# SensorsINI/v2e

Measured on NVIDIA H100. Metric: Mevents/s, higher is better.
Workload: dtype fp16 tensor-core convs (fp32 accumulate) + f64 pixel state

## Files before the change

### include/v2e_b200.h

```cpp
#ifndef V2E_B200_H
#define V2E_B200_H

#include <stdint.h>

#ifdef __cplusplus
extern "C" {
#endif

typedef enum V2eStatus {
    V2E_OK = 0,
    V2E_E_INVALID = -1,
    V2E_E_CUDA = -2,
    V2E_E_CAPACITY = -3,
    V2E_E_ITER_CAP = -4,
    V2E_E_STATE = -5,
    V2E_E_UNSUPPORTED = -6,
    V2E_E_FALLBACK = -7
} V2eStatus;

typedef enum V2eFrameDtype { V2E_U8 = 0, V2E_F32 = 1, V2E_F64 = 2 } V2eFrameDtype;

const char *v2e_last_error(void);
int v2e_version(void);
int v2e_abi_info(int *version, int *emu_cfg_size, int *frame_info_size, int *unet_weights_size);
// ... 131 lines not shown

int v2e_emu_state_is_f64(V2eEmu *h);
void *v2e_emu_state_ptr(V2eEmu *h, int which);

int v2e_emu_draw_noise(V2eEmu *h, uint32_t frame_index, float *leak_randn, float *shot_u01, float *pr_randn,
                       void *stream);


int v2e_conv2d_lrelu_sm100(const void *x1_dev, int C1, const void *x2_dev, int C2,
                           const void *wgt_dev, const float *bias_dev, int Cout_pad, int KH, int KW,
                           int N, int H, int W, void *out_dev, int out_cstride, int out_mode,
                           int co_real, float slope, void *stream);

enum {
    V2E_CONV_TILE_AUTO = -1,
    V2E_CONV_TILE_LEGACY = 0,
    V2E_CONV_TILE_256x128 = 1,
    V2E_CONV_TILE_128x256 = 2
};
int v2e_conv2d_lrelu_sm100_tile(const void *x1_dev, int C1, const void *x2_dev, int C2,
                                const void *wgt_dev, const float *bias_dev, int Cout_pad, int KH, int KW,
                                int N, int H, int W, void *out_dev, int out_cstride, int out_mode,
                                int co_real, float slope, int tile, void *stream);
int v2e_conv_pick_tile(int C1, int C2, int Cout_pad, int KH, int KW, int N, int H, int W, int n_sms);

int v2e_conv2d_lrelu_sm100_strip(const void *x1_dev, int C1, const void *x2_dev, int C2,
                                 const void *wgt_row_dev, const float *bias_dev, int Cout_pad, int KH,
                                 int KW, int N, int H, int W, void *out_dev, int out_cstride,
                                 int out_mode, int co_real, float slope, void *stream);
int v2e_conv_strip_pick_kc(int C1, int C2, int Cout_pad, int KH, int KW, int W);

enum {
    V2E_STRIP_CHAIN_AUTO = -1,
    V2E_STRIP_CHAIN_PAIRED = 0,
    V2E_STRIP_CHAIN_STACKED = 1
};
int v2e_conv2d_lrelu_sm100_strip_chain(const void *x1_dev, int C1, const void *x2_dev, int C2,
                                       const void *wgt_row_dev, const float *bias_dev, int Cout_pad, int KH,
                                       int KW, int N, int H, int W, void *out_dev, int out_cstride,
                                       int out_mode, int co_real, float slope, int chain, void *stream);
int v2e_conv_strip_pick_chain(int C1, int C2, int Cout_pad, int KH, int KW, int W);

int v2e_conv2d_up2_lrelu_sm100(const void *x_low_dev, int C, const void *wgt_fold_dev, const void *wgt_plain_dev,
                               const float *bias_dev, int Cout_pad, int N, int H_out, int W_out, void *out_dev,
                               int out_cstride, float slope, void *stream);
int v2e_conv_up2_fold_weights(const float *w_host, int cout, int cin, int Cout_pad, int C_pad, void *out_host);
// ... 89 lines not shown
```

### v2e_b200/_lib.py

```python
import ctypes
import os

from . import build as _build

_LIB = None


class V2eEmuCfg(ctypes.Structure):
    _fields_ = [
        ("width", ctypes.c_int32), ("height", ctypes.c_int32),
        ("per_pixel_thres", ctypes.c_int32), ("hdr", ctypes.c_int32),
        ("pos_thres_nominal", ctypes.c_double), ("neg_thres_nominal", ctypes.c_double),
        ("cutoff_hz", ctypes.c_double), ("leak_rate_hz", ctypes.c_double),
        ("leak_jitter_fraction", ctypes.c_double), ("refractory_period_s", ctypes.c_double),
        ("shot_noise_rate_hz", ctypes.c_double), ("shot_inten_factor", ctypes.c_double),
        ("rng_mode", ctypes.c_int32), ("iter_cap", ctypes.c_int32),
        ("seed", ctypes.c_uint64),
        ("csdvs", ctypes.c_int32), ("max_frames_per_step", ctypes.c_int32),
        ("cs_tau_p_s", ctypes.c_double), ("cs_tau_h_s", ctypes.c_double),
        ("scidvs", ctypes.c_int32), ("photoreceptor_noise", ctypes.c_int32),
        ("rng_pixel_offset", ctypes.c_uint32), ("full_frame_px", ctypes.c_uint32),
        ("own_row0", ctypes.c_int32), ("own_rows", ctypes.c_int32),
        ("cs_halo_rows", ctypes.c_int32), ("reserved1", ctypes.c_int32),
    ]
# ... 53 lines not shown
    "v2e_emu_first_frame": (_i, [_vp, _vp, _i, _d, _d, _vp]),
    "v2e_emu_step": (_i, [_vp, _vp, _i, _i, _vp, _d, _vp, _vp, _vp, _u64, _u64, _i, _i, _vp]),
    "v2e_emu_collect": (_i, [_vp, ctypes.POINTER(V2eFrameInfo), _i, ctypes.POINTER(_i),
                             ctypes.POINTER(_u64), _vp]),
    "v2e_emu_phase_count": (_i, [_vp, _vp, _i, _d, _d, _vp, _vp, _i, _u64, _u64, _vp]),
    "v2e_emu_phase_update": (_i, [_vp, _vp, _i, _d, _d, _vp, _vp, _u64, _u64, _vp]),
    "v2e_emu_max_n_dev": (_vp, [_vp]),
    "v2e_emu_cs_begin": (_i, [_vp, _vp, _i, _d, _d, _u64, _u64, ctypes.POINTER(_i), _vp]),
    "v2e_emu_cs_pack": (_i, [_vp, _vp]),
    "v2e_emu_cs_unpack_from": (_i, [_vp, _vp, _vp, _vp]),
    "v2e_emu_cs_send_dev": (_vp, [_vp]),
    "v2e_emu_cs_chunk": (_i, [_vp, _i, _i, _vp]),
    "v2e_emu_cs_max_dev": (_vp, [_vp]),
    "v2e_emu_cs_advance": (_i, [_vp, _i, _i, _vp]),
    "v2e_emu_cs_update": (_i, [_vp, _vp, _i, _vp, _vp, _vp]),
    "v2e_emu_phase_filter": (_i, [_vp, _d, _d, _u64, _i, _vp]),
    "v2e_emu_read_counts": (_i, [_vp, ctypes.POINTER(ctypes.c_int32), _vp, _i, _vp]),
    "v2e_emu_phase_shot": (_i, [_vp, _vp, _i, _d, _d, _vp, _u64, _vp]),
    "v2e_emu_phase_emit": (_i, [_vp, _d, _d, _vp, _u64, _vp]),
    "v2e_conv2d_lrelu_sm100": (_i, [_vp, _i, _vp, _i, _vp, _vp, _i, _i, _i, _i, _i, _i, _vp, _i, _i, _i,
                                    ctypes.c_float, _vp]),
    "v2e_conv2d_lrelu_sm100_tile": (_i, [_vp, _i, _vp, _i, _vp, _vp, _i, _i, _i, _i, _i, _i, _vp, _i, _i, _i,
                                         ctypes.c_float, _i, _vp]),
    "v2e_conv_pick_tile": (_i, [_i, _i, _i, _i, _i, _i, _i, _i, _i]),
    "v2e_conv2d_lrelu_sm100_strip": (_i, [_vp, _i, _vp, _i, _vp, _vp, _i, _i, _i, _i, _i, _i, _vp, _i, _i, _i,
                                          ctypes.c_float, _vp]),
    "v2e_conv_strip_pick_kc": (_i, [_i, _i, _i, _i, _i, _i]),
    "v2e_conv2d_lrelu_sm100_strip_chain": (_i, [_vp, _i, _vp, _i, _vp, _vp, _i, _i, _i, _i, _i, _i, _vp, _i, _i, _i,
                                                ctypes.c_float, _i, _vp]),
    "v2e_conv_strip_pick_chain": (_i, [_i, _i, _i, _i, _i, _i]),
    "v2e_conv2d_up2_lrelu_sm100": (_i, [_vp, _i, _vp, _vp, _vp, _i, _i, _i, _i, _vp, _i, ctypes.c_float, _vp]),
    "v2e_conv_up2_fold_weights": (_i, [_vp, _i, _i, _i, _i, _vp]),
    "v2e_conv_up2_supported_c": (_i, [_i, _i, _i]),
    "v2e_slomo_create": (_i, [_i, _i, _i, _vp, _vp, ctypes.POINTER(_vp)]),
    "v2e_slomo_destroy": (_i, [_vp]),
    "v2e_slomo_set_pairs": (_i, [_vp, _vp, _i, _vp]),
    "v2e_slomo_max_flow": (_i, [_vp, ctypes.POINTER(ctypes.c_float), _vp]),
    "v2e_slomo_interp": (_i, [_vp, _d, _vp, _vp, _vp]),
    "v2e_slomo_set_option": (_i, [_vp, _i, _i]),
    "v2e_slomo_check_finite": (_i, [_vp, ctypes.POINTER(_i), _vp]),
    "v2e_slomo_profile": (_i, [_vp, _i]),
    "v2e_slomo_profile_read": (_i, [_vp, ctypes.POINTER(ctypes.c_float), ctypes.POINTER(_i),
                                    ctypes.POINTER(ctypes.c_double), _vp]),
    "v2e_slomo_profile_read_layers": (_i, [_vp, ctypes.POINTER(ctypes.c_float), ctypes.POINTER(_i),
                                           ctypes.POINTER(ctypes.c_double), ctypes.POINTER(ctypes.c_float),
                                           ctypes.POINTER(_i), ctypes.POINTER(ctypes.c_double), _vp]),
# ... 98 lines not shown
```

### v2e_b200/csrc/conv_tc.cu

```cuda
#include <cuda.h>
#include <cuda_fp16.h>
#include <cuda_runtime.h>
#include <math.h>
#include <stdint.h>
#include <stdio.h>
#include <string.h>
#include <vector>

#include "../../include/v2e_b200.h"
#include "common.cuh"
#include "tc_common.cuh"

namespace {

constexpr int kTileH = 8, kTileW = 16, kBM = kTileH * kTileW;
constexpr int kStages = 4;
constexpr int kConvThreads = 288;
constexpr int kProducerWarp = 8;
constexpr int kConsumerWarps = 8;

struct ConvParams {
    int N, H, W;
    int C1, C2;
    int KH, KW;
    int KC;
    int BN;
    int stages;
    int co_fast;
    int tiles_x, tiles_y;
    int n_tiles;
    int out_cstride;
    int out_mode;
    int co_real;
    float slope;
    const float *bias;
    void *out;
};

__device__ __forceinline__ uint8_t *align1024(uint8_t *p) { return (uint8_t *)(((uintptr_t)p + 1023) & ~(uintptr_t)1023); }

__device__ __forceinline__ float lrelu(float x, float slope) { return x > 0.f ? x : x * slope; }

template <int BN>
__device__ __forceinline__ void epilogue_row(const float (&d)[BN / 2], int i, bool inb, size_t pix, int lane,
                                             const float *bias, float slope, int out_mode, void *out, int cstride,
                                             int co0, __half2 (&h)[BN / 8]) {
#pragma unroll
    for (int j = 0; j < BN / 8; j++) {
        const int c = 8 * j + 2 * (lane & 3);
        const float x0 = lrelu(d[4 * j + 2 * i] + __ldg(bias + c), slope);
        const float x1 = lrelu(d[4 * j + 2 * i + 1] + __ldg(bias + c + 1), slope);
        h[j] = __floats2half2_rn(x0, x1);
        if (inb) {
            if (out_mode == 0) *(__half2 *)((__half *)out + pix * cstride + co0 + c) = h[j];
            else if (j == 0) *(float2 *)((float *)out + pix * 8 + c) = make_float2(x0, x1);
        }
    }
}

template <int BN>
__global__ void __launch_bounds__(kConvThreads, 1)
conv_tc_kernel(const __grid_constant__ CUtensorMap tmA, const __grid_constant__ CUtensorMap tmA2,
               const __grid_constant__ CUtensorMap tmB, const ConvParams p) {
    extern __shared__ __align__(1024) uint8_t smem_raw[];
    uint8_t *smem = align1024(smem_raw);
    const uint32_t a_bytes = kBM * p.KC * 2;
    const uint32_t b_bytes_raw = BN * p.KC * 2;
    const uint32_t b_bytes = (b_bytes_raw + 1023) & ~1023u;
    const uint32_t stage_bytes = a_bytes + b_bytes;
    __shared__ __align__(8) uint64_t full_bar[kStages], empty_bar[kStages];

    const int warp = threadIdx.x >> 5, lane = threadIdx.x & 31;
    const int tile = p.co_fast ? blockIdx.y : blockIdx.x;
    const int tx = tile % p.tiles_x, ty = (tile / p.tiles_x) % p.tiles_y, n = tile / (p.tiles_x * p.tiles_y);
    const int x0 = tx * kTileW, y0 = ty * kTileH;
    const int n0 = (p.co_fast ? blockIdx.x : blockIdx.y) * BN;
    const int Ctot = p.C1 + p.C2;
    const int slabs = Ctot / p.KC;
    const int k_iters = p.KH * p.KW * slabs;

    if (threadIdx.x == 0) {
        for (int s = 0; s < kStages; s++) { mbar_init(&full_bar[s], 1); mbar_init(&empty_bar[s], kConsumerWarps); }
        fence_barrier_init();
    }
    if (warp == kProducerWarp && lane == 0) {
        prefetch_tmap(&tmA);
        if (p.C2) prefetch_tmap(&tmA2);
        prefetch_tmap(&tmB);
    }
    __syncthreads();

    if (warp == kProducerWarp) {
        if (lane == 0) {
            int stage = 0;
            uint32_t phase = 0;
            const int ph = p.KH / 2, pw = p.KW / 2;
            for (int tap = 0; tap < p.KH * p.KW; tap++) {
                const int r = tap / p.KW, s = tap % p.KW;
                for (int sl = 0; sl < slabs; sl++) {
                    mbar_wait(&empty_bar[stage], phase ^ 1);
                    uint8_t *sa = smem + stage * stage_bytes, *sb = sa + a_bytes;
                    mbar_expect_tx(&full_bar[stage], a_bytes + b_bytes_raw);
                    const int c = sl * p.KC;
                    if (c < p.C1) tma_load_4d(sa, &tmA, &full_bar[stage], c, x0 + s - pw, y0 + r - ph, n);
                    else tma_load_4d(sa, &tmA2, &full_bar[stage], c - p.C1, x0 + s - pw, y0 + r - ph, n);
                    tma_load_2d(sb, &tmB, &full_bar[stage], tap * Ctot + c, n0);
                    if (++stage == p.stages) { stage = 0; phase ^= 1; }
                }
            }
        }
    } else {
        const int g = warp >> 2;
        const uint64_t d0 = make_smem_desc(smem_u32(smem), swizzle_layout(p.KC), 8u * p.KC * 2u);
        const uint32_t stage16 = stage_bytes >> 4, a16 = a_bytes >> 4, half16 = (64u * p.KC * 2u) >> 4;
        const int ksteps = p.KC / 16;
        float acc[BN / 2];
#pragma unroll
        for (int i = 0; i < BN / 2; i++) acc[i] = 0.f;
        int stage = 0, prev = -1;
        uint32_t phase = 0;
        for (int it = 0; it < k_iters; it++) {
            mbar_wait(&full_bar[stage], phase);
            const uint32_t base = (uint32_t)stage * stage16;
            wgmma_fence();
            for (int j = 0; j < ksteps; j++)
                wgmma_f16<BN>(acc, desc_add(d0, base + (uint32_t)g * half16 + 2u * j), desc_add(d0, base + a16 + 2u * j),
                              (uint32_t)((it | j) != 0));
            wgmma_commit();
            wgmma_wait<1>();
            if (prev >= 0) { __syncwarp(); if (lane == 0) mbar_arrive(&empty_bar[prev]); }
            prev = stage;
            if (++stage == p.stages) { stage = 0; phase ^= 1; }
        }
        wgmma_wait<0>();
        wgmma_fence_regs(acc);
        __half2 hv[BN / 8];
#pragma unroll
        for (int i = 0; i < 2; i++) {
            const int m = 64 * g + 16 * (warp & 3) + (lane >> 2) + 8 * i;
            const int py = y0 + m / kTileW, px = x0 + m % kTileW;
            const bool inb = py < p.H && px < p.W;
            const size_t pix = ((size_t)n * p.H + py) * p.W + px;
            epilogue_row<BN>(acc, i, inb, pix, lane, p.bias + n0, p.slope, p.out_mode, p.out, p.out_cstride, n0, hv);
        }
    }
}

template <int MH, int BN>
__global__ void __launch_bounds__(kConvThreads, 1)
conv_wide_kernel(const __grid_constant__ CUtensorMap tmA, const __grid_constant__ CUtensorMap tmA2,
                 const __grid_constant__ CUtensorMap tmB, const ConvParams p) {
    constexpr int TH = kTileH * MH, BM = kBM * MH;
    extern __shared__ __align__(1024) uint8_t smem_raw[];
    uint8_t *smem = align1024(smem_raw);
    const uint32_t a_bytes = BM * p.KC * 2;
    const uint32_t b_bytes = BN * p.KC * 2;
    const uint32_t stage_bytes = a_bytes + b_bytes;
    __shared__ __align__(8) uint64_t full_bar[kStages], empty_bar[kStages];

    const int warp = threadIdx.x >> 5, lane = threadIdx.x & 31;
    const int tile = p.co_fast ? blockIdx.y : blockIdx.x;
    const int tx = tile % p.tiles_x, ty = (tile / p.tiles_x) % p.tiles_y, n = tile / (p.tiles_x * p.tiles_y);
    const int x0 = tx * kTileW, y0 = ty * TH;
    const int n0 = (p.co_fast ? blockIdx.x : blockIdx.y) * BN;
    const int Ctot = p.C1 + p.C2;
    const int slabs = Ctot / p.KC;
    const int k_iters = p.KH * p.KW * slabs;

    if (threadIdx.x == 0) {
        for (int s = 0; s < kStages; s++) { mbar_init(&full_bar[s], 1); mbar_init(&empty_bar[s], kConsumerWarps); }
        fence_barrier_init();
    }
    if (warp == kProducerWarp && lane == 0) {
        prefetch_tmap(&tmA);
        if (p.C2) prefetch_tmap(&tmA2);
        prefetch_tmap(&tmB);
    }
    __syncthreads();

    if (warp == kProducerWarp) {
        if (lane == 0) {
            int stage = 0;
            uint32_t phase = 0;
            const int ph = p.KH / 2, pw = p.KW / 2;
            for (int tap = 0; tap < p.KH * p.KW; tap++) {
                const int r = tap / p.KW, s = tap % p.KW;
                for (int sl = 0; sl < slabs; sl++) {
                    mbar_wait(&empty_bar[stage], phase ^ 1);
                    uint8_t *sa = smem + stage * stage_bytes, *sb = sa + a_bytes;
                    mbar_expect_tx(&full_bar[stage], a_bytes + b_bytes);
                    const int c = sl * p.KC;
                    if (c < p.C1) tma_load_4d(sa, &tmA, &full_bar[stage], c, x0 + s - pw, y0 + r - ph, n);
                    else tma_load_4d(sa, &tmA2, &full_bar[stage], c - p.C1, x0 + s - pw, y0 + r - ph, n);
                    tma_load_2d(sb, &tmB, &full_bar[stage], tap * Ctot + c, n0);
                    if (++stage == p.stages) { stage = 0; phase ^= 1; }
                }
            }
        }
    } else {
        const int g = __shfl_sync(0xffffffffu, warp >> 2, 0);
        const uint64_t d0 = make_smem_desc(smem_u32(smem), swizzle_layout(p.KC), 8u * p.KC * 2u);
        const uint32_t stage16 = stage_bytes >> 4, a16 = a_bytes >> 4, q16 = (64u * p.KC * 2u) >> 4;
        const int ksteps = p.KC / 16;
        float acc[MH][BN / 2];
#pragma unroll
        for (int h = 0; h < MH; h++) {
#pragma unroll
            for (int i = 0; i < BN / 2; i++) acc[h][i] = 0.f;
            wgmma_fence_regs(acc[h]);
        }
        int stage = 0, prev = -1;
        uint32_t phase = 0;
        for (int it = 0; it < k_iters; it++) {
            mbar_wait(&full_bar[stage], phase);
            const uint32_t base = (uint32_t)stage * stage16;
            wgmma_fence();
            for (int j = 0; j < ksteps; j++) {
#pragma unroll
                for (int h = 0; h < MH; h++)
                    wgmma_f16<BN>(acc[h], desc_add(d0, base + (uint32_t)(g * MH + h) * q16 + 2u * j),
                                  desc_add(d0, base + a16 + 2u * j), (uint32_t)((it | j) != 0));
            }
            wgmma_commit();
            wgmma_wait<1>();
            if (prev >= 0) { __syncwarp(); if (lane == 0) mbar_arrive(&empty_bar[prev]); }
            prev = stage;
            if (++stage == p.stages) { stage = 0; phase ^= 1; }
        }
        wgmma_wait<0>();
#pragma unroll
        for (int h = 0; h < MH; h++) wgmma_fence_regs(acc[h]);
        const float *bias = p.bias + n0;
        __half *out = (__half *)p.out + n0;
#pragma unroll
        for (int h = 0; h < MH; h++) {
            size_t pix[2];
            bool inb[2];
#pragma unroll
            for (int i = 0; i < 2; i++) {
                const int m = 64 * (g * MH + h) + 16 * (warp & 3) + (lane >> 2) + 8 * i;
                const int py = y0 + m / kTileW, px = x0 + m % kTileW;
                inb[i] = py < p.H && px < p.W;
                pix[i] = (((size_t)n * p.H + py) * p.W + px) * p.out_cstride;
            }
#pragma unroll
            for (int j = 0; j < BN / 8; j++) {
                const int c = 8 * j + 2 * (lane & 3);
                const float2 b = __ldg((const float2 *)(bias + c));
#pragma unroll
                for (int i = 0; i < 2; i++)
                    if (inb[i])
                        *(__half2 *)(out + pix[i] + c) = __floats2half2_rn(lrelu(acc[h][4 * j + 2 * i] + b.x, p.slope),
                                                                           lrelu(acc[h][4 * j + 2 * i + 1] + b.y, p.slope));
            }
        }
    }
}


constexpr int kRowTile = 128;

struct StripParams {
    int N, H, W;
    int C1, C2;
    int KH, KW;
    int KC, BN;
    int tiles_x, seg_h, n_seg, n_items;
    int nslot;
    void *pool_out;
    int pool_cstride;
    int n_split, cout_pad;
    int slab_bytes;
    int w_bytes;
    int out_cstride, out_mode, co_real;
    float slope;
    const float *bias;
    void *out;
};
constexpr int kMaxSlot = 12;
constexpr int kStripThreads = 288;

// ... 507 lines not shown
    const int kc = v2e_conv_pick_kc(C1, C2);
    if (n_sms < 1) n_sms = 1;
    int best = V2E_CONV_TILE_LEGACY;
    double best_cost = 0.0;
    for (int tile = V2E_CONV_TILE_LEGACY; tile <= V2E_CONV_TILE_128x256; tile++) {
        int mh, bn;
        tile_shape(tile, Cout_pad, &mh, &bn);
        const bool wide = tile != V2E_CONV_TILE_LEGACY;
        if (wide && (kc != 64 || Cout_pad % bn || (tile == V2E_CONV_TILE_256x128) != (Cout_pad == 128))) continue;
        long tiles = (long)((W + kTileW - 1) / kTileW) * ((H + kTileH * mh - 1) / (kTileH * mh)) * N;
        const long ctas = tiles * (Cout_pad / bn);
        const long waves = (ctas + n_sms - 1) / n_sms;
        const double a_bytes = (double)kBM * mh * kc * 2, b_bytes = (double)bn * kc * 2;
        const double flops = 2.0 * kBM * mh * bn * kc;
        const double per_stage = fmax((a_bytes + b_bytes) / 24.0, flops / 4096.0);
        const double cost = (double)waves * per_stage;
        if (tile == V2E_CONV_TILE_LEGACY || cost < best_cost) { best = tile; best_cost = cost; }
    }
    return best;
}

struct V2eConvLaunch {
    CUtensorMap tmA, tmA2, tmB;
    ConvParams p;
    dim3 grid;
    int mh;
    size_t smem;
};

int v2e_conv_prepare(V2eConvLaunch *L, const void *x1, int C1, const void *x2, int C2, const void *wgt,
                     const float *bias, int Cout_pad, int KH, int KW, int N, int H, int W, void *out,
                     int out_cstride, int out_mode, int co_real, float slope, int tile, int n_sms) {
    if (C1 % 16 || C2 % 16 || !(Cout_pad == 16 || Cout_pad == 32 || Cout_pad == 64 || (Cout_pad > 0 && Cout_pad % 128 == 0)))
        return v2e_set_error(V2E_E_INVALID, "conv: channel counts must be padded to 16 (Cout to 16/32/64/128k)%s", "");
    if (tile == V2E_CONV_TILE_AUTO) tile = v2e_conv_pick_tile(C1, C2, Cout_pad, KH, KW, N, H, W, n_sms);
    if (tile < V2E_CONV_TILE_LEGACY || tile > V2E_CONV_TILE_128x256)
        return v2e_set_error(V2E_E_INVALID, "conv: unknown tile%s", "");
    memset(L, 0, sizeof(*L));
    ConvParams &p = L->p;
    int mh, bn;
    tile_shape(tile, Cout_pad, &mh, &bn);
    const bool wide = tile != V2E_CONV_TILE_LEGACY;
    p.N = N; p.H = H; p.W = W; p.C1 = C1; p.C2 = C2; p.KH = KH; p.KW = KW;
    p.KC = v2e_conv_pick_kc(C1, C2);
    p.BN = bn;
    if (wide && (Cout_pad % bn || out_mode != 0))
        return v2e_set_error(V2E_E_INVALID, "conv: the wide tiles need fp16 output and Cout_pad a multiple of their width%s", "");
    p.stages = kStages;
    p.tiles_x = (W + kTileW - 1) / kTileW;
    p.tiles_y = (H + kTileH * mh - 1) / (kTileH * mh);
    p.n_tiles = p.tiles_x * p.tiles_y * N;
    p.out_cstride = out_cstride; p.out_mode = out_mode; p.co_real = co_real; p.slope = slope;
    p.bias = bias; p.out = out;
    L->mh = mh;
    int rc;
    if ((rc = make_act_tmap_h(&L->tmA, x1, N, H, W, C1, p.KC, kTileH * mh))) return rc;
    if (C2) { if ((rc = make_act_tmap_h(&L->tmA2, x2, N, H, W, C2, p.KC, kTileH * mh))) return rc; }
    else L->tmA2 = L->tmA;
    if ((rc = v2e_make_wgt_tmap(&L->tmB, wgt, Cout_pad, KH * KW * (C1 + C2), p.KC, bn))) return rc;
    const unsigned tiles = (unsigned)p.n_tiles, cob = (unsigned)(Cout_pad / p.BN);
    p.co_fast = (cob > 1 && tiles <= 65535u) ? 1 : 0;
    L->grid = p.co_fast ? dim3(cob, tiles, 1) : dim3(tiles, cob, 1);
    size_t stage = (size_t)kBM * mh * p.KC * 2 + (((size_t)p.BN * p.KC * 2 + 1023) & ~(size_t)1023);
    L->smem = stage * p.stages + 1024;
    return V2E_OK;
}

template <int BN>
static cudaError_t conv_launch_bn(const V2eConvLaunch *L, cudaStream_t st) {
    static PerDeviceOnce attr_once;
    if (attr_once.first()) cudaFuncSetAttribute(conv_tc_kernel<BN>, cudaFuncAttributeMaxDynamicSharedMemorySize, 200 * 1024);
    conv_tc_kernel<BN><<<L->grid, kConvThreads, L->smem, st>>>(L->tmA, L->tmA2, L->tmB, L->p);
    return cudaGetLastError();
}

template <int MH, int BN>
static cudaError_t conv_launch_wide(const V2eConvLaunch *L, cudaStream_t st) {
    static PerDeviceOnce attr_once;
    if (attr_once.first())
        cudaFuncSetAttribute(conv_wide_kernel<MH, BN>, cudaFuncAttributeMaxDynamicSharedMemorySize, 226 * 1024);
    conv_wide_kernel<MH, BN><<<L->grid, kConvThreads, L->smem, st>>>(L->tmA, L->tmA2, L->tmB, L->p);
    return cudaGetLastError();
}

int v2e_conv_launch(const V2eConvLaunch *L, cudaStream_t st) {
    cudaError_t e;
    if (L->mh == 2 && L->p.BN == 128) e = conv_launch_wide<2, 128>(L, st);
    else if (L->mh == 1 && L->p.BN == 256) e = conv_launch_wide<1, 256>(L, st);
    else switch (L->p.BN) {
        case 16: e = conv_launch_bn<16>(L, st); break;
        case 32: e = conv_launch_bn<32>(L, st); break;
        case 64: e = conv_launch_bn<64>(L, st); break;
        case 128: e = conv_launch_bn<128>(L, st); break;
        default: return v2e_set_error(V2E_E_UNSUPPORTED, "conv_tc_kernel: unsupported tile width%s", "");
    }
    if (e != cudaSuccess) return v2e_set_error(V2E_E_CUDA, "conv_tc_kernel launch: %s", cudaGetErrorString(e));
    return V2E_OK;
}

size_t v2e_conv_launch_size(void) { return sizeof(V2eConvLaunch); }

static int device_sms() {
    int dev = 0, sms = 132;
    cudaGetDevice(&dev);
    cudaDeviceGetAttribute(&sms, cudaDevAttrMultiProcessorCount, dev);
    return sms;
}

extern "C" int v2e_conv2d_lrelu_sm100_tile(const void *x1_dev, int C1, const void *x2_dev, int C2,
                                           const void *wgt_dev, const float *bias_dev, int Cout_pad, int KH, int KW,
                                           int N, int H, int W, void *out_dev, int out_cstride, int out_mode,
                                           int co_real, float slope, int tile, void *stream) {
    V2eConvLaunch L;
    int rc = v2e_conv_prepare(&L, x1_dev, C1, x2_dev, C2, wgt_dev, bias_dev, Cout_pad, KH, KW, N, H, W, out_dev,
                              out_cstride, out_mode, co_real, slope, tile, device_sms());
    if (rc) return rc;
    return v2e_conv_launch(&L, (cudaStream_t)stream);
}

extern "C" int v2e_conv2d_lrelu_sm100(const void *x1_dev, int C1, const void *x2_dev, int C2,
                                      const void *wgt_dev, const float *bias_dev, int Cout_pad, int KH, int KW,
                                      int N, int H, int W, void *out_dev, int out_cstride, int out_mode,
                                      int co_real, float slope, void *stream) {
    return v2e_conv2d_lrelu_sm100_tile(x1_dev, C1, x2_dev, C2, wgt_dev, bias_dev, Cout_pad, KH, KW, N, H, W, out_dev,
                                       out_cstride, out_mode, co_real, slope, V2E_CONV_TILE_AUTO, stream);
}

struct V2eStripLaunch {
    CUtensorMap tmA, tmA2, tmB;
    StripParams p;
    int stacked;
    int grid;
    size_t smem;
};

static int make_rowseg_tmap(CUtensorMap *tm, const void *ptr, int N, int H, int W, int C, int KC, int KW) {
    EncodeTiledFn fn = encode_fn();
    if (!fn) return v2e_set_error(V2E_E_CUDA, "cuTensorMapEncodeTiled unavailable%s", "");
    cuuint64_t dims[4] = {(cuuint64_t)C, (cuuint64_t)W, (cuuint64_t)H, (cuuint64_t)N};
    cuuint64_t strides[3] = {(cuuint64_t)C * 2, (cuuint64_t)W * C * 2, (cuuint64_t)H * W * C * 2};
// ... 336 lines not shown
```

### v2e_b200/csrc/tc_common.cuh

```cuda
#pragma once
#include <cuda.h>
#include <cuda_runtime.h>
#include <stdint.h>

__device__ __forceinline__ uint32_t smem_u32(const void *p) { return (uint32_t)__cvta_generic_to_shared(p); }

__device__ __forceinline__ void mbar_init(uint64_t *bar, uint32_t count) {
    asm volatile("mbarrier.init.shared::cta.b64 [%0], %1;" ::"r"(smem_u32(bar)), "r"(count) : "memory");
}
__device__ __forceinline__ void fence_barrier_init() { asm volatile("fence.mbarrier_init.release.cluster;" ::: "memory"); }
__device__ __forceinline__ void fence_proxy_async() { asm volatile("fence.proxy.async.shared::cta;" ::: "memory"); }
__device__ __forceinline__ void mbar_expect_tx(uint64_t *bar, uint32_t bytes) {
    asm volatile("mbarrier.arrive.expect_tx.shared::cta.b64 _, [%0], %1;" ::"r"(smem_u32(bar)), "r"(bytes) : "memory");
}
__device__ __forceinline__ void mbar_arrive(uint64_t *bar) {
    asm volatile("mbarrier.arrive.shared::cta.b64 _, [%0];" ::"r"(smem_u32(bar)) : "memory");
}
__device__ __forceinline__ void mbar_wait(uint64_t *bar, uint32_t parity) {
    const uint32_t addr = smem_u32(bar);
    uint32_t done;
    do {
        asm volatile(
            "{\n\t.reg .pred p;\n\t"
            "mbarrier.try_wait.parity.shared::cta.b64 p, [%1], %2;\n\t"
            "selp.u32 %0, 1, 0, p;\n\t}"
            : "=r"(done) : "r"(addr), "r"(parity) : "memory");
    } while (!done);
}

__device__ __forceinline__ void prefetch_tmap(const CUtensorMap *tm) {
    asm volatile("prefetch.tensormap [%0];" ::"l"((uint64_t)tm) : "memory");
}
__device__ __forceinline__ void tma_load_4d(void *dst, const CUtensorMap *tm, uint64_t *bar, int c0, int c1, int c2, int c3) {
    asm volatile(
        "cp.async.bulk.tensor.4d.shared::cluster.global.tile.mbarrier::complete_tx::bytes [%0], [%1, {%3, %4, %5, %6}], [%2];"
        ::"r"(smem_u32(dst)), "l"((uint64_t)tm), "r"(smem_u32(bar)), "r"(c0), "r"(c1), "r"(c2), "r"(c3) : "memory");
}
__device__ __forceinline__ void tma_load_2d(void *dst, const CUtensorMap *tm, uint64_t *bar, int c0, int c1) {
    asm volatile(
        "cp.async.bulk.tensor.2d.shared::cluster.global.tile.mbarrier::complete_tx::bytes [%0], [%1, {%3, %4}], [%2];"
        ::"r"(smem_u32(dst)), "l"((uint64_t)tm), "r"(smem_u32(bar)), "r"(c0), "r"(c1) : "memory");
}

__device__ __forceinline__ uint32_t elect_one() {
    uint32_t pred;
    asm volatile("{\n\t.reg .pred p;\n\telect.sync _|p, 0xffffffff;\n\tselp.u32 %0, 1, 0, p;\n\t}" : "=r"(pred));
    return pred;
}

__device__ __forceinline__ void wgmma_fence() { asm volatile("wgmma.fence.sync.aligned;" ::: "memory"); }
__device__ __forceinline__ void wgmma_commit() { asm volatile("wgmma.commit_group.sync.aligned;" ::: "memory"); }
template <int N>
__device__ __forceinline__ void wgmma_wait() { asm volatile("wgmma.wait_group.sync.aligned %0;" ::"n"(N) : "memory"); }
template <int R>
__device__ __forceinline__ void wgmma_fence_regs(float (&d)[R]) {
#pragma unroll
    for (int i = 0; i < R; i++) asm volatile("" : "+f"(d[i])::"memory");
}

__device__ __forceinline__ void wgmma_m64n16k16(float (&d)[8], uint64_t adesc, uint64_t bdesc, uint32_t scale_d) {
    asm volatile(
        "{\n\t.reg .pred p;\n\tsetp.ne.b32 p, %10, 0;\n\t"
        "wgmma.mma_async.sync.aligned.m64n16k16.f32.f16.f16 {%0, %1, %2, %3, %4, %5, %6, %7}, %8, %9, p, 1, 1, 0, 0;\n\t}"
        : "+f"(d[0]), "+f"(d[1]), "+f"(d[2]), "+f"(d[3]), "+f"(d[4]), "+f"(d[5]), "+f"(d[6]), "+f"(d[7])
        : "l"(adesc), "l"(bdesc), "r"(scale_d) : "memory");
}
__device__ __forceinline__ void wgmma_m64n32k16(float (&d)[16], uint64_t adesc, uint64_t bdesc, uint32_t scale_d) {
    asm volatile(
        "{\n\t.reg .pred p;\n\tsetp.ne.b32 p, %18, 0;\n\t"
        "wgmma.mma_async.sync.aligned.m64n32k16.f32.f16.f16 {%0, %1, %2, %3, %4, %5, %6, %7, %8, %9, %10, %11, %12, %13, %14, %15}, %16, %17, p, 1, 1, 0, 0;\n\t}"
        : "+f"(d[0]), "+f"(d[1]), "+f"(d[2]), "+f"(d[3]), "+f"(d[4]), "+f"(d[5]), "+f"(d[6]), "+f"(d[7]), "+f"(d[8]), "+f"(d[9]), "+f"(d[10]), "+f"(d[11]), "+f"(d[12]), "+f"(d[13]), "+f"(d[14]), "+f"(d[15])
// ... 43 lines not shown
```

Measured before the change: 56.85.

## Make conv kernels persistent and store wide-tile epilogue through swizzled TMA

Both conv kernels become persistent. The grid is capped at the SM count, and each CTA walks tiles times output-channel blocks while keeping the mbarrier ring phase across items, so the next tile's loads overlap the current epilogue. The wide kernel moves to a full producer warpgroup of 384 threads, uses setmaxnreg to shift registers to the consumers, and writes fp16 output by staging it in swizzled shared memory and issuing TMA bulk stores instead of scattered half2 stores. This adds shared memory for staging and new alignment requirements on the output stride, and it removes per-launch tile scheduling.

```diff
diff --git a/include/v2e_b200.h b/include/v2e_b200.h
--- a/include/v2e_b200.h
+++ b/include/v2e_b200.h
@@ -177,6 +177,10 @@
                                 const void *wgt_dev, const float *bias_dev, int Cout_pad, int KH, int KW,
                                 int N, int H, int W, void *out_dev, int out_cstride, int out_mode,
                                 int co_real, float slope, int tile, void *stream);
+int v2e_conv2d_lrelu_sm100_plan(const void *x1_dev, int C1, const void *x2_dev, int C2,
+                                const void *wgt_dev, const float *bias_dev, int Cout_pad, int KH, int KW,
+                                int N, int H, int W, void *out_dev, int out_cstride, int out_mode,
+                                int co_real, float slope, int tile, int n_sms, void *stream);
 int v2e_conv_pick_tile(int C1, int C2, int Cout_pad, int KH, int KW, int N, int H, int W, int n_sms);
 
 int v2e_conv2d_lrelu_sm100_strip(const void *x1_dev, int C1, const void *x2_dev, int C2,
diff --git a/v2e_b200/_lib.py b/v2e_b200/_lib.py
--- a/v2e_b200/_lib.py
+++ b/v2e_b200/_lib.py
@@ -99,6 +99,8 @@
                                     ctypes.c_float, _vp]),
     "v2e_conv2d_lrelu_sm100_tile": (_i, [_vp, _i, _vp, _i, _vp, _vp, _i, _i, _i, _i, _i, _i, _vp, _i, _i, _i,
                                          ctypes.c_float, _i, _vp]),
+    "v2e_conv2d_lrelu_sm100_plan": (_i, [_vp, _i, _vp, _i, _vp, _vp, _i, _i, _i, _i, _i, _i, _vp, _i, _i, _i,
+                                         ctypes.c_float, _i, _i, _vp]),
     "v2e_conv_pick_tile": (_i, [_i, _i, _i, _i, _i, _i, _i, _i, _i]),
     "v2e_conv2d_lrelu_sm100_strip": (_i, [_vp, _i, _vp, _i, _vp, _vp, _i, _i, _i, _i, _i, _i, _vp, _i, _i, _i,
                                           ctypes.c_float, _vp]),
diff --git a/v2e_b200/csrc/conv_tc.cu b/v2e_b200/csrc/conv_tc.cu
--- a/v2e_b200/csrc/conv_tc.cu
+++ b/v2e_b200/csrc/conv_tc.cu
@@ -18,6 +18,9 @@
 constexpr int kConvThreads = 288;
 constexpr int kProducerWarp = 8;
 constexpr int kConsumerWarps = 8;
+constexpr int kWideThreads = 384;
+constexpr int kWideProducerRegs = 40, kWideConsumerRegs = 232;
+constexpr uint32_t kWideStageBytes = 64 * 128 * 2;
 
 struct ConvParams {
     int N, H, W;
@@ -26,9 +29,10 @@
     int KC;
     int BN;
     int stages;
-    int co_fast;
     int tiles_x, tiles_y;
     int n_tiles;
+    int cob;
+    int n_items;
     int out_cstride;
     int out_mode;
     int co_real;
@@ -56,6 +60,66 @@
             else if (j == 0) *(float2 *)((float *)out + pix * 8 + c) = make_float2(x0, x1);
         }
     }
+}
+
+struct TapItem {
+    int x0, y0, n, n0;
+};
+__device__ __forceinline__ TapItem tap_item(const ConvParams &p, int w, int tile_h, int bn) {
+    const int tile = w / p.cob;
+    const int tx = tile % p.tiles_x, ty = (tile / p.tiles_x) % p.tiles_y;
+    return {tx * kTileW, ty * tile_h, tile / (p.tiles_x * p.tiles_y), (w % p.cob) * bn};
+}
+
+struct RingPos {
+    int stage;
+    uint32_t phase;
+    __device__ __forceinline__ void next(int stages) { if (++stage == stages) { stage = 0; phase ^= 1; } }
+};
+
+__device__ __forceinline__ void tap_producer(const CUtensorMap *tmA, const CUtensorMap *tmA2, const CUtensorMap *tmB,
+                                             const ConvParams &p, uint8_t *smem, uint32_t a_bytes, uint32_t stage_bytes,
+                                             uint32_t tx_bytes, int tile_h, int bn, uint64_t *full_bar,
+                                             uint64_t *empty_bar) {
+    const int Ctot = p.C1 + p.C2, slabs = Ctot / p.KC;
+    const int ph = p.KH / 2, pw = p.KW / 2;
+    RingPos rp{0, 0};
+    for (int w = blockIdx.x; w < p.n_items; w += gridDim.x) {
+        const TapItem t = tap_item(p, w, tile_h, bn);
+        for (int tap = 0; tap < p.KH * p.KW; tap++) {
+            const int r = tap / p.KW, s = tap % p.KW;
+            for (int sl = 0; sl < slabs; sl++) {
+                mbar_wait(&empty_bar[rp.stage], rp.phase ^ 1);
+                uint8_t *sa = smem + rp.stage * stage_bytes, *sb = sa + a_bytes;
+                mbar_expect_tx(&full_bar[rp.stage], tx_bytes);
+                const int c = sl * p.KC;
+                if (c < p.C1) tma_load_4d(sa, tmA, &full_bar[rp.stage], c, t.x0 + s - pw, t.y0 + r - ph, t.n);
+                else tma_load_4d(sa, tmA2, &full_bar[rp.stage], c - p.C1, t.x0 + s - pw, t.y0 + r - ph, t.n);
+                tma_load_2d(sb, tmB, &full_bar[rp.stage], tap * Ctot + c, t.n0);
+                rp.next(p.stages);
+            }
+        }
+    }
+}
+
+__device__ __forceinline__ void tap_ring_init(const CUtensorMap *tmA, const CUtensorMap *tmA2, const CUtensorMap *tmB,
+                                              const ConvParams &p, uint64_t *full_bar, uint64_t *empty_bar) {
+    const int warp = threadIdx.x >> 5, lane = threadIdx.x & 31;
+    if (threadIdx.x == 0) {
+        for (int s = 0; s < kStages; s++) { mbar_init(&full_bar[s], 1); mbar_init(&empty_bar[s], kConsumerWarps); }
+        fence_barrier_init();
+    }
+    if (warp == kProducerWarp && lane == 0) {
+        prefetch_tmap(tmA);
+        if (p.C2) prefetch_tmap(tmA2);
+        prefetch_tmap(tmB);
+    }
+    __syncthreads();
+}
+
+__device__ __forceinline__ void release_stage(uint64_t *empty_bar, int stage, int lane) {
+    __syncwarp();
+    if (lane == 0) mbar_arrive(&empty_bar[stage]);
 }
 
 template <int BN>
@@ -71,85 +135,59 @@
     __shared__ __align__(8) uint64_t full_bar[kStages], empty_bar[kStages];
 
     const int warp = threadIdx.x >> 5, lane = threadIdx.x & 31;
-    const int tile = p.co_fast ? blockIdx.y : blockIdx.x;
-    const int tx = tile % p.tiles_x, ty = (tile / p.tiles_x) % p.tiles_y, n = tile / (p.tiles_x * p.tiles_y);
-    const int x0 = tx * kTileW, y0 = ty * kTileH;
-    const int n0 = (p.co_fast ? blockIdx.x : blockIdx.y) * BN;
-    const int Ctot = p.C1 + p.C2;
-    const int slabs = Ctot / p.KC;
-    const int k_iters = p.KH * p.KW * slabs;
-
-    if (threadIdx.x == 0) {
-        for (int s = 0; s < kStages; s++) { mbar_init(&full_bar[s], 1); mbar_init(&empty_bar[s], kConsumerWarps); }
-        fence_barrier_init();
-    }
-    if (warp == kProducerWarp && lane == 0) {
-        prefetch_tmap(&tmA);
-        if (p.C2) prefetch_tmap(&tmA2);
-        prefetch_tmap(&tmB);
-    }
-    __syncthreads();
+    const int k_iters = p.KH * p.KW * ((p.C1 + p.C2) / p.KC);
+    tap_ring_init(&tmA, &tmA2, &tmB, p, full_bar, empty_bar);
 
     if (warp == kProducerWarp) {
-        if (lane == 0) {
-            int stage = 0;
-            uint32_t phase = 0;
-            const int ph = p.KH / 2, pw = p.KW / 2;
-            for (int tap = 0; tap < p.KH * p.KW; tap++) {
-                const int r = tap / p.KW, s = tap % p.KW;
-                for (int sl = 0; sl < slabs; sl++) {
-                    mbar_wait(&empty_bar[stage], phase ^ 1);
-                    uint8_t *sa = smem + stage * stage_bytes, *sb = sa + a_bytes;
-                    mbar_expect_tx(&full_bar[stage], a_bytes + b_bytes_raw);
-                    const int c = sl * p.KC;
-                    if (c < p.C1) tma_load_4d(sa, &tmA, &full_bar[stage], c, x0 + s - pw, y0 + r - ph, n);
-                    else tma_load_4d(sa, &tmA2, &full_bar[stage], c - p.C1, x0 + s - pw, y0 + r - ph, n);
-                    tma_load_2d(sb, &tmB, &full_bar[stage], tap * Ctot + c, n0);
-                    if (++stage == p.stages) { stage = 0; phase ^= 1; }
-                }
-            }
-        }
+        if (lane == 0)
+            tap_producer(&tmA, &tmA2, &tmB, p, smem, a_bytes, stage_bytes, a_bytes + b_bytes_raw, kTileH, BN, full_bar,
+                         empty_bar);
     } else {
         const int g = warp >> 2;
         const uint64_t d0 = make_smem_desc(smem_u32(smem), swizzle_layout(p.KC), 8u * p.KC * 2u);
         const uint32_t stage16 = stage_bytes >> 4, a16 = a_bytes >> 4, half16 = (64u * p.KC * 2u) >> 4;
         const int ksteps = p.KC / 16;
-        float acc[BN / 2];
-#pragma unroll
-        for (int i = 0; i < BN / 2; i++) acc[i] = 0.f;
-        int stage = 0, prev = -1;
-        uint32_t phase = 0;
-        for (int it = 0; it < k_iters; it++) {
-            mbar_wait(&full_bar[stage], phase);
-            const uint32_t base = (uint32_t)stage * stage16;
-            wgmma_fence();
-            for (int j = 0; j < ksteps; j++)
-                wgmma_f16<BN>(acc, desc_add(d0, base + (uint32_t)g * half16 + 2u * j), desc_add(d0, base + a16 + 2u * j),
-                              (uint32_t)((it | j) != 0));
-            wgmma_commit();
-            wgmma_wait<1>();
-            if (prev >= 0) { __syncwarp(); if (lane == 0) mbar_arrive(&empty_bar[prev]); }
-            prev = stage;
-            if (++stage == p.stages) { stage = 0; phase ^= 1; }
+        RingPos rp{0, 0};
+        for (int w = blockIdx.x; w < p.n_items; w += gridDim.x) {
+            float acc[BN / 2];
+#pragma unroll
+            for (int i = 0; i < BN / 2; i++) acc[i] = 0.f;
+            int prev = -1;
+            for (int it = 0; it < k_iters; it++) {
+                mbar_wait(&full_bar[rp.stage], rp.phase);
+                const uint32_t base = (uint32_t)rp.stage * stage16;
+                wgmma_fence();
+                for (int j = 0; j < ksteps; j++)
+                    wgmma_f16<BN>(acc, desc_add(d0, base + (uint32_t)g * half16 + 2u * j), desc_add(d0, base + a16 + 2u * j),
+                                  (uint32_t)((it | j) != 0));
+                wgmma_commit();
+                wgmma_wait<1>();
+                if (prev >= 0) release_stage(empty_bar, prev, lane);
+                prev = rp.stage;
+                rp.next(p.stages);
+            }
+            wgmma_wait<0>();
+            release_stage(empty_bar, prev, lane);
+            wgmma_fence_regs(acc);
+            const TapItem t = tap_item(p, w, kTileH, BN);
+            __half2 hv[BN / 8];
+#pragma unroll
+            for (int i = 0; i < 2; i++) {
+                const int m = 64 * g + 16 * (warp & 3) + (lane >> 2) + 8 * i;
+                const int py = t.y0 + m / kTileW, px = t.x0 + m % kTileW;
+                const bool inb = py < p.H && px < p.W;
+                const size_t pix = ((size_t)t.n * p.H + py) * p.W + px;
+                epilogue_row<BN>(acc, i, inb, pix, lane, p.bias + t.n0, p.slope, p.out_mode, p.out, p.out_cstride, t.n0,
+                                 hv);
+            }
         }
-        wgmma_wait<0>();
-        wgmma_fence_regs(acc);
-        __half2 hv[BN / 8];
-#pragma unroll
-        for (int i = 0; i < 2; i++) {
-            const int m = 64 * g + 16 * (warp & 3) + (lane >> 2) + 8 * i;
-            const int py = y0 + m / kTileW, px = x0 + m % kTileW;
-            const bool inb = py < p.H && px < p.W;
-            const size_t pix = ((size_t)n * p.H + py) * p.W + px;
-            epilogue_row<BN>(acc, i, inb, pix, lane, p.bias + n0, p.slope, p.out_mode, p.out, p.out_cstride, n0, hv);
-        }
     }
 }
 
 template <int MH, int BN>
-__global__ void __launch_bounds__(kConvThreads, 1)
+__global__ void __launch_bounds__(kWideThreads, 1)
 conv_wide_kernel(const __grid_constant__ CUtensorMap tmA, const __grid_constant__ CUtensorMap tmA2,
-                 const __grid_constant__ CUtensorMap tmB, const ConvParams p) {
+                 const __grid_constant__ CUtensorMap tmB, const __grid_constant__ CUtensorMap tmC, const ConvParams p) {
     constexpr int TH = kTileH * MH, BM = kBM * MH;
     extern __shared__ __align__(1024) uint8_t smem_raw[];
     uint8_t *smem = align1024(smem_raw);
@@ -159,104 +197,84 @@
     __shared__ __align__(8) uint64_t full_bar[kStages], empty_bar[kStages];
 
     const int warp = threadIdx.x >> 5, lane = threadIdx.x & 31;
-    const int tile = p.co_fast ? blockIdx.y : blockIdx.x;
-    const int tx = tile % p.tiles_x, ty = (tile / p.tiles_x) % p.tiles_y, n = tile / (p.tiles_x * p.tiles_y);
-    const int x0 = tx * kTileW, y0 = ty * TH;
-    const int n0 = (p.co_fast ? blockIdx.x : blockIdx.y) * BN;
-    const int Ctot = p.C1 + p.C2;
-    const int slabs = Ctot / p.KC;
-    const int k_iters = p.KH * p.KW * slabs;
-
-    if (threadIdx.x == 0) {
-        for (int s = 0; s < kStages; s++) { mbar_init(&full_bar[s], 1); mbar_init(&empty_bar[s], kConsumerWarps); }
-        fence_barrier_init();
-    }
-    if (warp == kProducerWarp && lane == 0) {
-        prefetch_tmap(&tmA);
-        if (p.C2) prefetch_tmap(&tmA2);
-        prefetch_tmap(&tmB);
-    }
-    __syncthreads();
-
-    if (warp == kProducerWarp) {
-        if (lane == 0) {
-            int stage = 0;
-            uint32_t phase = 0;
-            const int ph = p.KH / 2, pw = p.KW / 2;
-            for (int tap = 0; tap < p.KH * p.KW; tap++) {
-                const int r = tap / p.KW, s = tap % p.KW;
-                for (int sl = 0; sl < slabs; sl++) {
-                    mbar_wait(&empty_bar[stage], phase ^ 1);
-                    uint8_t *sa = smem + stage * stage_bytes, *sb = sa + a_bytes;
-                    mbar_expect_tx(&full_bar[stage], a_bytes + b_bytes);
-                    const int c = sl * p.KC;
-                    if (c < p.C1) tma_load_4d(sa, &tmA, &full_bar[stage], c, x0 + s - pw, y0 + r - ph, n);
-                    else tma_load_4d(sa, &tmA2, &full_bar[stage], c - p.C1, x0 + s - pw, y0 + r - ph, n);
-                    tma_load_2d(sb, &tmB, &full_bar[stage], tap * Ctot + c, n0);
-                    if (++stage == p.stages) { stage = 0; phase ^= 1; }
-                }
-            }
-        }
+    const int k_iters = p.KH * p.KW * ((p.C1 + p.C2) / p.KC);
+    tap_ring_init(&tmA, &tmA2, &tmB, p, full_bar, empty_bar);
+
+    if (warp >= kProducerWarp) {
+        setmaxnreg_dec<kWideProducerRegs>();
+        if (warp == kProducerWarp && lane == 0)
+            tap_producer(&tmA, &tmA2, &tmB, p, smem, a_bytes, stage_bytes, a_bytes + b_bytes, TH, BN, full_bar, empty_bar);
     } else {
+        setmaxnreg_inc<kWideConsumerRegs>();
+        if ((threadIdx.x & 127) == 0) prefetch_tmap(&tmC);
         const int g = __shfl_sync(0xffffffffu, warp >> 2, 0);
         const uint64_t d0 = make_smem_desc(smem_u32(smem), swizzle_layout(p.KC), 8u * p.KC * 2u);
         const uint32_t stage16 = stage_bytes >> 4, a16 = a_bytes >> 4, q16 = (64u * p.KC * 2u) >> 4;
         const int ksteps = p.KC / 16;
-        float acc[MH][BN / 2];
-#pragma unroll
-        for (int h = 0; h < MH; h++) {
-#pragma unroll
-            for (int i = 0; i < BN / 2; i++) acc[h][i] = 0.f;
-            wgmma_fence_regs(acc[h]);
+        RingPos rp{0, 0};
+        for (int w = blockIdx.x; w < p.n_items; w += gridDim.x) {
+            float acc[MH][BN / 2];
+#pragma unroll
+            for (int h = 0; h < MH; h++) {
+#pragma unroll
+                for (int i = 0; i < BN / 2; i++) acc[h][i] = 0.f;
+                wgmma_fence_regs(acc[h]);
+            }
+            int prev = -1;
+            for (int it = 0; it < k_iters; it++) {
+                mbar_wait(&full_bar[rp.stage], rp.phase);
+                const uint32_t base = (uint32_t)rp.stage * stage16;
+                wgmma_fence();
+                for (int j = 0; j < ksteps; j++) {
+#pragma unroll
+                    for (int h = 0; h < MH; h++)
+                        wgmma_f16<BN>(acc[h], desc_add(d0, base + (uint32_t)(g * MH + h) * q16 + 2u * j),
+                                      desc_add(d0, base + a16 + 2u * j), (uint32_t)((it | j) != 0));
+                }
+                wgmma_commit();
+                wgmma_wait<1>();
+                if (prev >= 0) release_stage(empty_bar, prev, lane);
+                prev = rp.stage;
+                rp.next(p.stages);
+            }
+            wgmma_wait<0>();
+            release_stage(empty_bar, prev, lane);
+#pragma unroll
+            for (int h = 0; h < MH; h++) wgmma_fence_regs(acc[h]);
+            const TapItem t = tap_item(p, w, TH, BN);
+            const bool leader = (threadIdx.x & 127) == 0;
+            uint8_t *stg = smem + (size_t)p.stages * stage_bytes + (size_t)g * kWideStageBytes;
+            const int r = lane >> 2;
+#pragma unroll
+            for (int c = 0; c < 2; c++) {
+                const int h = MH == 2 ? c : 0, k = MH == 2 ? 0 : c;
+                if (leader) bulk_wait_group_read<0>();
+                named_bar_sync(1 + g, 128);
+#pragma unroll
+                for (int jj = 0; jj < 16; jj++) {
+                    const int j = 16 * k + jj;
+                    const float2 b = __ldg((const float2 *)(p.bias + t.n0 + 8 * j + 2 * (lane & 3)));
+#pragma unroll
+                    for (int i = 0; i < 2; i++) {
+                        const int m = 16 * (warp & 3) + r + 8 * i;
+                        *(__half2 *)(stg + (jj >> 3) * 8192 + m * 128 + (((jj & 7) ^ r) << 4) + 4 * (lane & 3)) =
+                            __floats2half2_rn(lrelu(acc[h][4 * j + 2 * i] + b.x, p.slope),
+                                              lrelu(acc[h][4 * j + 2 * i + 1] + b.y, p.slope));
+                    }
+                }
+                fence_proxy_async();
+                named_bar_sync(1 + g, 128);
+                if (leader) {
+                    const int y = t.y0 + 4 * (g * MH + h), co = t.n0 + 128 * k;
+                    tma_store_4d(&tmC, stg, co, t.x0, y, t.n);
+                    tma_store_4d(&tmC, stg + 8192, co + 64, t.x0, y, t.n);
+                    bulk_commit_group();
+                }
+            }
         }
-        int stage = 0, prev = -1;
-        uint32_t phase = 0;
-        for (int it = 0; it < k_iters; it++) {
-            mbar_wait(&full_bar[stage], phase);
-            const uint32_t base = (uint32_t)stage * stage16;
-            wgmma_fence();
-            for (int j = 0; j < ksteps; j++) {
-#pragma unroll
-                for (int h = 0; h < MH; h++)
-                    wgmma_f16<BN>(acc[h], desc_add(d0, base + (uint32_t)(g * MH + h) * q16 + 2u * j),
-                                  desc_add(d0, base + a16 + 2u * j), (uint32_t)((it | j) != 0));
-            }
-            wgmma_commit();
-            wgmma_wait<1>();
-            if (prev >= 0) { __syncwarp(); if (lane == 0) mbar_arrive(&empty_bar[prev]); }
-            prev = stage;
-            if (++stage == p.stages) { stage = 0; phase ^= 1; }
-        }
-        wgmma_wait<0>();
-#pragma unroll
-        for (int h = 0; h < MH; h++) wgmma_fence_regs(acc[h]);
-        const float *bias = p.bias + n0;
-        __half *out = (__half *)p.out + n0;
-#pragma unroll
-        for (int h = 0; h < MH; h++) {
-            size_t pix[2];
-            bool inb[2];
-#pragma unroll
-            for (int i = 0; i < 2; i++) {
-                const int m = 64 * (g * MH + h) + 16 * (warp & 3) + (lane >> 2) + 8 * i;
-                const int py = y0 + m / kTileW, px = x0 + m % kTileW;
-                inb[i] = py < p.H && px < p.W;
-                pix[i] = (((size_t)n * p.H + py) * p.W + px) * p.out_cstride;
-            }
-#pragma unroll
-            for (int j = 0; j < BN / 8; j++) {
-                const int c = 8 * j + 2 * (lane & 3);
-                const float2 b = __ldg((const float2 *)(bias + c));
-#pragma unroll
-                for (int i = 0; i < 2; i++)
-                    if (inb[i])
-                        *(__half2 *)(out + pix[i] + c) = __floats2half2_rn(lrelu(acc[h][4 * j + 2 * i] + b.x, p.slope),
-                                                                           lrelu(acc[h][4 * j + 2 * i + 1] + b.y, p.slope));
-            }
-        }
-    }
-}
-
+        if ((threadIdx.x & 127) == 0) bulk_wait_group<0>();
+    }
+}
 
 constexpr int kRowTile = 128;
 
@@ -810,6 +828,7 @@
 
 struct V2eConvLaunch {
     CUtensorMap tmA, tmA2, tmB;
+    CUtensorMap tmC;
     ConvParams p;
     dim3 grid;
     int mh;
@@ -834,6 +853,9 @@
     p.BN = bn;
     if (wide && (Cout_pad % bn || out_mode != 0))
         return v2e_set_error(V2E_E_INVALID, "conv: the wide tiles need fp16 output and Cout_pad a multiple of their width%s", "");
+    if (wide && (out_cstride % 8 || (uintptr_t)out % 16))
+        return v2e_set_error(V2E_E_INVALID, "conv: the wide tiles store by TMA: out_cstride must be a multiple of 8 and the "
+                             "output 16-byte aligned%s", "");
     p.stages = kStages;
     p.tiles_x = (W + kTileW - 1) / kTileW;
     p.tiles_y = (H + kTileH * mh - 1) / (kTileH * mh);
@@ -846,11 +868,24 @@
     if (C2) { if ((rc = make_act_tmap_h(&L->tmA2, x2, N, H, W, C2, p.KC, kTileH * mh))) return rc; }
     else L->tmA2 = L->tmA;
     if ((rc = v2e_make_wgt_tmap(&L->tmB, wgt, Cout_pad, KH * KW * (C1 + C2), p.KC, bn))) return rc;
-    const unsigned tiles = (unsigned)p.n_tiles, cob = (unsigned)(Cout_pad / p.BN);
-    p.co_fast = (cob > 1 && tiles <= 65535u) ? 1 : 0;
-    L->grid = p.co_fast ? dim3(cob, tiles, 1) : dim3(tiles, cob, 1);
+    if (wide) {
+        EncodeTiledFn fn = encode_fn();
+        cuuint64_t dims[4] = {(cuuint64_t)out_cstride, (cuuint64_t)W, (cuuint64_t)H, (cuuint64_t)N};
+        cuuint64_t strides[3] = {(cuuint64_t)out_cstride * 2, (cuuint64_t)W * out_cstride * 2,
+                                 (cuuint64_t)H * W * out_cstride * 2};
+        cuuint32_t box[4] = {64, (cuuint32_t)kTileW, 4, 1};
+        cuuint32_t es[4] = {1, 1, 1, 1};
+        CUresult r = fn(&L->tmC, CU_TENSOR_MAP_DATA_TYPE_FLOAT16, 4, out, dims, strides, box, es,
+                        CU_TENSOR_MAP_INTERLEAVE_NONE, CU_TENSOR_MAP_SWIZZLE_128B, CU_TENSOR_MAP_L2_PROMOTION_L2_256B,
+                        CU_TENSOR_MAP_FLOAT_OOB_FILL_NONE);
+        if (r != CUDA_SUCCESS) return v2e_set_error(V2E_E_CUDA, "cuTensorMapEncodeTiled failed for the output map%s", "");
+    }
+    p.cob = Cout_pad / p.BN;
+    p.n_items = p.n_tiles * p.cob;
+    const int sms = n_sms < 1 ? 1 : n_sms;
+    L->grid = dim3(p.n_items < sms ? p.n_items : sms, 1, 1);
     size_t stage = (size_t)kBM * mh * p.KC * 2 + (((size_t)p.BN * p.KC * 2 + 1023) & ~(size_t)1023);
-    L->smem = stage * p.stages + 1024;
+    L->smem = stage * p.stages + 1024 + (wide ? 2 * (size_t)kWideStageBytes : 0);
     return V2E_OK;
 }
 
@@ -867,7 +902,7 @@
     static PerDeviceOnce attr_once;
     if (attr_once.first())
         cudaFuncSetAttribute(conv_wide_kernel<MH, BN>, cudaFuncAttributeMaxDynamicSharedMemorySize, 226 * 1024);
-    conv_wide_kernel<MH, BN><<<L->grid, kConvThreads, L->smem, st>>>(L->tmA, L->tmA2, L->tmB, L->p);
+    conv_wide_kernel<MH, BN><<<L->grid, kWideThreads, L->smem, st>>>(L->tmA, L->tmA2, L->tmB, L->tmC, L->p);
     return cudaGetLastError();
 }
 
@@ -895,15 +930,23 @@
     return sms;
 }
 
+extern "C" int v2e_conv2d_lrelu_sm100_plan(const void *x1_dev, int C1, const void *x2_dev, int C2,
+                                           const void *wgt_dev, const float *bias_dev, int Cout_pad, int KH, int KW,
+                                           int N, int H, int W, void *out_dev, int out_cstride, int out_mode,
+                                           int co_real, float slope, int tile, int n_sms, void *stream) {
+    V2eConvLaunch L;
+    int rc = v2e_conv_prepare(&L, x1_dev, C1, x2_dev, C2, wgt_dev, bias_dev, Cout_pad, KH, KW, N, H, W, out_dev,
+                              out_cstride, out_mode, co_real, slope, tile, n_sms);
+    if (rc) return rc;
+    return v2e_conv_launch(&L, (cudaStream_t)stream);
+}
+
 extern "C" int v2e_conv2d_lrelu_sm100_tile(const void *x1_dev, int C1, const void *x2_dev, int C2,
                                            const void *wgt_dev, const float *bias_dev, int Cout_pad, int KH, int KW,
                                            int N, int H, int W, void *out_dev, int out_cstride, int out_mode,
                                            int co_real, float slope, int tile, void *stream) {
-    V2eConvLaunch L;
-    int rc = v2e_conv_prepare(&L, x1_dev, C1, x2_dev, C2, wgt_dev, bias_dev, Cout_pad, KH, KW, N, H, W, out_dev,
-                              out_cstride, out_mode, co_real, slope, tile, device_sms());
-    if (rc) return rc;
-    return v2e_conv_launch(&L, (cudaStream_t)stream);
+    return v2e_conv2d_lrelu_sm100_plan(x1_dev, C1, x2_dev, C2, wgt_dev, bias_dev, Cout_pad, KH, KW, N, H, W, out_dev,
+                                       out_cstride, out_mode, co_real, slope, tile, device_sms(), stream);
 }
 
 extern "C" int v2e_conv2d_lrelu_sm100(const void *x1_dev, int C1, const void *x2_dev, int C2,
diff --git a/v2e_b200/csrc/tc_common.cuh b/v2e_b200/csrc/tc_common.cuh
--- a/v2e_b200/csrc/tc_common.cuh
+++ b/v2e_b200/csrc/tc_common.cuh
@@ -41,12 +41,29 @@
         "cp.async.bulk.tensor.2d.shared::cluster.global.tile.mbarrier::complete_tx::bytes [%0], [%1, {%3, %4}], [%2];"
         ::"r"(smem_u32(dst)), "l"((uint64_t)tm), "r"(smem_u32(bar)), "r"(c0), "r"(c1) : "memory");
 }
+__device__ __forceinline__ void tma_store_4d(const CUtensorMap *tm, const void *src, int c0, int c1, int c2, int c3) {
+    asm volatile("cp.async.bulk.tensor.4d.global.shared::cta.bulk_group [%0, {%2, %3, %4, %5}], [%1];"
+                 ::"l"((uint64_t)tm), "r"(smem_u32(src)), "r"(c0), "r"(c1), "r"(c2), "r"(c3) : "memory");
+}
+__device__ __forceinline__ void bulk_commit_group() { asm volatile("cp.async.bulk.commit_group;" ::: "memory"); }
+template <int N>
+__device__ __forceinline__ void bulk_wait_group_read() { asm volatile("cp.async.bulk.wait_group.read %0;" ::"n"(N) : "memory"); }
+template <int N>
+__device__ __forceinline__ void bulk_wait_group() { asm volatile("cp.async.bulk.wait_group %0;" ::"n"(N) : "memory"); }
+__device__ __forceinline__ void named_bar_sync(int id, int count) {
+    asm volatile("bar.sync %0, %1;" ::"r"(id), "r"(count) : "memory");
+}
 
 __device__ __forceinline__ uint32_t elect_one() {
     uint32_t pred;
     asm volatile("{\n\t.reg .pred p;\n\telect.sync _|p, 0xffffffff;\n\tselp.u32 %0, 1, 0, p;\n\t}" : "=r"(pred));
     return pred;
 }
+
+template <int N>
+__device__ __forceinline__ void setmaxnreg_dec() { asm volatile("setmaxnreg.dec.sync.aligned.u32 %0;" ::"n"(N)); }
+template <int N>
+__device__ __forceinline__ void setmaxnreg_inc() { asm volatile("setmaxnreg.inc.sync.aligned.u32 %0;" ::"n"(N)); }
 
 __device__ __forceinline__ void wgmma_fence() { asm volatile("wgmma.fence.sync.aligned;" ::: "memory"); }
 __device__ __forceinline__ void wgmma_commit() { asm volatile("wgmma.commit_group.sync.aligned;" ::: "memory"); }
```

After: 59.44, median of 6. 1.05x the previous value.
